# marcin-ochman/modular-slam

Measured on AMD Instinct MI355X. Metric: ORB keypoints extracted+matched /sec, 640×480 RGB-D, 1/2/4/8 GPU; HBM GB/s vs roofline, higher is better.
Workload: dtype u8

## Files before the change

modular-slam_amd/csrc/api.hip:

```cpp
#include "context.hpp"

#include <cfloat>
#include <climits>
#include <cmath>
#include <cstdio>
#include <cstring>
#include <cstdlib>
#include <algorithm>

using namespace mslam;

static thread_local std::string g_create_error;

#define ENTER(c)                                                                                                       \
    do                                                                                                                 \
    {                                                                                                                  \
        if(!(c))                                                                                                       \
            return MSLAM_HIP_E_INVALID;                                                                                \
        MSLAM_CHK(c, hipSetDevice((c)->p.device));                                                                     \
    } while(0)

static inline int cv_round_f(float v) { return (int)lrintf(v); }
static inline int cv_floor_f(float v)
{
// ... 1224 lines not shown
                exec = nullptr;
            if(rc)
                return rc;
            MSLAM_CHK(c, e);
            MSLAM_CHK(c, e_inst);
        }
        MSLAM_CHK(c, hipGraphLaunch(exec, c->stream));
    }
    else
    {
        rc = enqueue_detect(c, frame_src, 1);
        if(rc)
            return rc;
        rc = enqueue_results();
        if(rc)
            return rc;
    }
    MSLAM_CHK(c, hipEventRecord(c->out[c->cur].ev_detect, c->stream));
    c->n_last = 1;
    ++c->detect_seq;
    MSLAM_CHK(c, hipStreamSynchronize(c->stream));
    uint32_t flags;
    int32_t n;
    std::memcpy(&n, h, 4);
    std::memcpy(&flags, h + 4, 4);
    if(flags)
        return check_flags(c);
    *n_out = n;
    if(n > max_out)
        return fail(c, MSLAM_HIP_E_CAPACITY, "detect: max_out smaller than the number of keypoints");
    if(n == 0)
        return MSLAM_HIP_OK;
    std::memcpy(xy, h_xy, (size_t)n * 8);
    std::memcpy(desc, h_desc, (size_t)n * 32);
    if(octave)
        std::memcpy(octave, h_oct, (size_t)n * 4);
    if(angle)
        std::memcpy(angle, h_ang, (size_t)n * 4);
    if(response)
        std::memcpy(response, h_resp, (size_t)n * 4);
    return MSLAM_HIP_OK;
}

static int upload_ratio_table(mslam_hip_ctx* c, double ratio)
{
    if(ratio == c->ratio_cached)
        return MSLAM_HIP_OK;
    int32_t thr[257];
    for(int d1 = 0; d1 <= 256; ++d1)
    {
        int n = 0;
        for(int d0 = 0; d0 <= 256; ++d0)
            if((double)(float)d0 < ratio * (double)(float)d1)
                ++n;
            else
                break;
        thr[d1] = n;
    }
    MSLAM_CHK(c, hipStreamSynchronize(c->stream_m));
    MSLAM_CHK(c, hipMemcpyAsync(c->d_ratio_thr, thr, sizeof(thr), hipMemcpyHostToDevice, c->stream));
    MSLAM_CHK(c, hipStreamSynchronize(c->stream));
    c->ratio_cached = ratio;
    return MSLAM_HIP_OK;
}
__attribute__((visibility("hidden"))) int mslam_ratio_table(mslam_hip_ctx* c, double ratio) { return upload_ratio_table(c, ratio); }

int mslam_hip_match_batch_dev(mslam_hip_ctx* c, double ratio, int chain_previous)
{
    ENTER(c);
    if(c->n_last < 1)
        return fail(c, MSLAM_HIP_E_INVALID, "match_batch_dev: no detect batch to match");
    int rc = upload_ratio_table(c, ratio);
    if(rc)
        return rc;
    const size_t K = (size_t)c->p.max_keypoints;
    const int first = (chain_previous && c->have_prev) ? 0 : 1;
    const int n_pairs = c->n_last - first;
    c->match_seq = c->detect_seq;
    const bool own = c->overlap_match && !c->profiling;
    hipStream_t s = own ? c->stream_m : c->stream;
    if(own)
        MSLAM_CHK(c, hipStreamWaitEvent(s, c->out[c->cur].ev_detect, 0));
    if(first == 1)
        MSLAM_CHK(c, hipMemsetAsync(cur_out(c).mcount, 0, 4, s));
    if(n_pairs > 0)
    {
        MatchArgs m{};
        m.from_desc = cur_out(c).desc + (size_t)(first + 1) * K * 32;
        m.to_desc = cur_out(c).desc + (size_t)first * K * 32;
        m.from_stride = m.to_stride = (long long)K * 32;
        m.from_cnt = cur_out(c).count + first + 1;
        m.to_cnt = cur_out(c).count + first;
        m.cap = c->p.max_keypoints;
        m.cap_from = c->p.max_keypoints;
        m.popcount_only = c->matcher_kind == MSLAM_HIP_MATCHER_POPCOUNT;
        m.idx0 = cur_out(c).idx0 + (size_t)first * K;
        m.idx1 = cur_out(c).idx1 + (size_t)first * K;
        m.dist0 = cur_out(c).dist0 + (size_t)first * K;
        m.dist1 = cur_out(c).dist1 + (size_t)first * K;
        {
            StageScope t(c, "match_knn2", s);
            c->last_match_kernel = launch_match_knn2(m, n_pairs, s);
        }
        RatioArgs r{};
        r.idx0 = m.idx0;
        r.dist0 = m.dist0;
        r.dist1 = m.dist1;
        r.from_cnt = m.from_cnt;
        r.to_cnt = m.to_cnt;
        r.cap = m.cap;
        r.thr = c->d_ratio_thr;
        r.from_idx = cur_out(c).mfrom + (size_t)first * K;
        r.to_idx = cur_out(c).mto + (size_t)first * K;
        r.n_out = cur_out(c).mcount + first;
        {
            StageScope t(c, "ratio_compact", s);
            launch_ratio_compact(r, n_pairs, s);
        }
    }
    MSLAM_CHK(c, hipGetLastError());
    if(own)
    {
        MSLAM_CHK(c, hipEventRecord(c->out[c->cur].ev_match, s));
        c->out[c->cur].match_pending = true;
    }
    return MSLAM_HIP_OK;
}

constexpr int kHostMatchSlices = 8;
static int host_match_prepare(mslam_hip_ctx* c, const uint8_t* from_desc, int n_from, const uint8_t* to_desc, int n_to)
{
    if(n_from > c->hm_from_cap || n_to > c->hm_to_cap)
    {
        MSLAM_CHK(c, hipStreamSynchronize(c->stream));
        const int from_cap = std::max(n_from, std::max(c->hm_from_cap, 2048)), to_cap = std::max(n_to, std::max(c->hm_to_cap, 2048));
        c->hm_from_cap = c->hm_to_cap = 0;
        c->d_hm_to = nullptr;
        if(c->match_graph)
        {
            (void)hipGraphExecDestroy(c->match_graph);
            c->match_graph = nullptr;
        }
        MSLAM_CHK(c, c->d_hm_from.alloc((size_t)(from_cap + to_cap) * 32 + 16));
        MSLAM_CHK(c, c->d_hm_out.alloc((size_t)to_cap * 6 + 4));
        MSLAM_CHK(c, c->d_hm_partial.alloc((size_t)kHostMatchSlices * 2 * to_cap));
        MSLAM_CHK(c, c->h_hm.alloc((size_t)(from_cap + to_cap) * 32 + 16 + ((size_t)to_cap * 2 + 4) * 4));
        c->hm_from_cap = from_cap;
        c->hm_to_cap = to_cap;
    }
    c->d_hm_to = c->d_hm_from + (size_t)n_from * 32;
    if(n_from > 0)
        std::memcpy(c->h_hm, from_desc, (size_t)n_from * 32);
    std::memcpy(c->h_hm + (size_t)n_from * 32, to_desc, (size_t)n_to * 32);
    MSLAM_CHK(c, hipMemcpyAsync(c->d_hm_from, c->h_hm, (size_t)(n_from + n_to) * 32, hipMemcpyHostToDevice, c->stream));
    return MSLAM_HIP_OK;
}

static void host_match_args(mslam_hip_ctx* c, int n_from, int n_to, MatchArgs& m)
{
    const size_t cap = (size_t)c->hm_to_cap;
    m = MatchArgs{};
    m.from_desc = c->d_hm_from;
    m.to_desc = c->d_hm_to;
    m.n_from_fixed = n_from;
    m.n_to_fixed = n_to;
    m.cap = n_to;
    m.idx0 = c->d_hm_out;
// ... 388 lines not shown
```

modular-slam_amd/csrc/k_points.hip:

```cpp
#include "reloc.hpp"

#include <cfloat>

namespace mslam
{

struct Camera
{
    double cx, cy, inv_fx, inv_fy;
    float factor;
};

__global__ __launch_bounds__(256) void k_backproject(const uint16_t* __restrict__ depth, long long depth_stride, int w, int h,
                                                     Camera cam, const float* __restrict__ xy, long long xy_stride,
                                                     const int32_t* __restrict__ counts, int n_fixed, int cap,
                                                     double* __restrict__ xyz, uint8_t* __restrict__ valid)
{
    const int frame = blockIdx.y;
    const int n = min(counts ? counts[frame] : n_fixed, cap);
    const int i = blockIdx.x * 256 + threadIdx.x;
    if(i >= n)
        return;
    const float* p = xy + frame * xy_stride + 2 * (size_t)i;
    const double x = (double)p[0], y = (double)p[1];
    const bool inside = (x > -1.0) & (x < (double)w) & (y > -1.0) & (y < (double)h);
    float d = 0.f;
    if(inside)
        d = __fmul_rn((float)depth[frame * depth_stride + (size_t)w * (int)y + (int)x], cam.factor);
    const bool ok = d > FLT_EPSILON;
    const size_t o = (size_t)frame * cap + i;
    const double z = (double)d;
    xyz[3 * o] = ok ? (x - cam.cx) * z * cam.inv_fx : 0.0;
    xyz[3 * o + 1] = ok ? (y - cam.cy) * z * cam.inv_fy : 0.0;
    xyz[3 * o + 2] = ok ? z : 0.0;
    valid[o] = ok ? 1 : 0;
}

void launch_backproject(hipStream_t s, const uint16_t* d_depth, int width, int height, float factor, double fx, double fy, double cx,
                        double cy, const float* d_xy, int n, double* d_xyz, uint8_t* d_valid)
{
    const Camera cam{cx, cy, 1.0 / fx, 1.0 / fy, factor};
    hipLaunchKernelGGL(k_backproject, dim3((n + 255) / 256, 1), dim3(256), 0, s, d_depth, 0ll, width, height, cam, d_xy, 0ll, nullptr, n,
                       n, d_xyz, d_valid);
}

void launch_backproject_batch(hipStream_t s, const uint16_t* d_depth, int width, int height, float factor, double fx, double fy,
                              double cx, double cy, const float* d_xy, const int32_t* d_n, int stride, int n_frames, double* d_xyz,
                              uint8_t* d_valid)
{
    const Camera cam{cx, cy, 1.0 / fx, 1.0 / fy, factor};
    hipLaunchKernelGGL(k_backproject, dim3((stride + 255) / 256, n_frames), dim3(256), 0, s, d_depth, (long long)width * height, width,
                       height, cam, d_xy, (long long)stride * 2, d_n, 0, stride, d_xyz, d_valid);
}

}

using namespace mslam;

__global__ __launch_bounds__(1024) void k_pack_plan(const int32_t* __restrict__ count, const int32_t* __restrict__ mcount, int n_frames,
                                                    int cap, int with_points, unsigned long long capacity_bytes, uint8_t* __restrict__ out,
                                                    uint32_t* __restrict__ flags)
{
    __shared__ uint32_t wsum[2][16];
    __shared__ uint32_t carry[2];
    const int tid = threadIdx.x, lane = tid & 63, wave = tid >> 6;
    mslam_hip_packed_header* h = reinterpret_cast<mslam_hip_packed_header*>(out);
    const unsigned long long hdr = (sizeof(mslam_hip_packed_header) + 15) & ~15ull;
    const unsigned long long tab = (((unsigned long long)(n_frames + 1) * 4) + 15) & ~15ull;
    const bool room_for_tables = capacity_bytes >= hdr + 2 * tab;
    int32_t* kp_off = reinterpret_cast<int32_t*>(out + hdr);
    int32_t* m_off = reinterpret_cast<int32_t*>(out + hdr + tab);
    if(tid < 2)
        carry[tid] = 0;
    __syncthreads();
    for(int base = 0; base < n_frames; base += 1024)
    {
        const int t = base + tid;
        uint32_t v[2] = {t < n_frames ? (uint32_t)min(max(count[t], 0), cap) : 0u, (t < n_frames && mcount) ? (uint32_t)min(max(mcount[t], 0), cap) : 0u};
        uint32_t inc[2];
#pragma unroll
        for(int k = 0; k < 2; ++k)
        {
            uint32_t x = v[k];
            for(int o = 1; o < 64; o <<= 1)
            {
                const uint32_t y = (uint32_t)__shfl_up((int)x, o);
                x += lane >= o ? y : 0u;
            }
            inc[k] = x;
            if(lane == 63)
                wsum[k][wave] = x;
        }
        __syncthreads();
#pragma unroll
        for(int k = 0; k < 2; ++k)
        {
            uint32_t pre = carry[k];
            for(int w = 0; w < wave; ++w)
                pre += wsum[k][w];
            if(t < n_frames && room_for_tables)
                (k == 0 ? kp_off : m_off)[t] = (int32_t)(pre + inc[k] - v[k]);
        }
        __syncthreads();
        if(tid < 2)
        {
            uint32_t tot = carry[tid];
            for(int w = 0; w < 16; ++w)
                tot += wsum[tid][w];
            carry[tid] = tot;
        }
        __syncthreads();
    }
    if(tid == 0)
    {
        const unsigned long long nk = carry[0], nm = carry[1];
        auto al = [](unsigned long long x) { return (x + 15) & ~15ull; };
        unsigned long long o = hdr + 2 * tab;
        mslam_hip_packed_header hh;
        hh.n_frames = n_frames, hh.total_keypoints = (int32_t)nk, hh.total_matches = (int32_t)nm, hh.with_points = with_points;
        hh.off_kp_offset = hdr, hh.off_match_offset = hdr + tab;
        hh.off_xy = o, o = al(o + nk * 8);
        hh.off_desc = o, o = al(o + nk * 32);
        hh.off_octave = o, o = al(o + nk * 4);
        hh.off_angle = o, o = al(o + nk * 4);
        hh.off_response = o, o = al(o + nk * 4);
        hh.off_xyz = o, o = al(o + (with_points ? nk * 24 : 0));
        hh.off_valid = o, o = al(o + (with_points ? nk : 0));
        hh.off_match_from = o, o = al(o + nm * 4);
        hh.off_match_to = o, o = al(o + nm * 4);
        hh.bytes = o;
        hh.fits = o <= capacity_bytes ? 1 : 0;
        hh.pad = 0;
        if(capacity_bytes >= sizeof(hh))
            *h = hh;
// ... 4 lines not shown
    }
}

__global__ __launch_bounds__(256) void k_pack_copy(const float* __restrict__ xy, const uint8_t* __restrict__ desc, const int32_t* __restrict__ octave,
                                                   const float* __restrict__ angle, const float* __restrict__ response,
                                                   const double* __restrict__ xyz, const uint8_t* __restrict__ valid,
                                                   const int32_t* __restrict__ mfrom, const int32_t* __restrict__ mto, int cap,
                                                   uint8_t* __restrict__ out)
{
    const mslam_hip_packed_header* h = reinterpret_cast<const mslam_hip_packed_header*>(out);
    if(!h->fits)
        return;
    const int t = blockIdx.x, tid = blockIdx.y * 256 + threadIdx.x, nt = gridDim.y * 256;
    const int32_t* kp_off = reinterpret_cast<const int32_t*>(out + h->off_kp_offset);
    const int32_t* m_off = reinterpret_cast<const int32_t*>(out + h->off_match_offset);
    const size_t k0 = (size_t)kp_off[t], m0 = (size_t)m_off[t];
    const int n = kp_off[t + 1] - kp_off[t], m = m_off[t + 1] - m_off[t];
    const size_t f = (size_t)t * cap;
    uint2* o_xy = reinterpret_cast<uint2*>(out + h->off_xy) + k0;
    uint2* o_desc = reinterpret_cast<uint2*>(out + h->off_desc) + 4 * k0;
    uint32_t* o_oct = reinterpret_cast<uint32_t*>(out + h->off_octave) + k0;
    uint32_t* o_ang = reinterpret_cast<uint32_t*>(out + h->off_angle) + k0;
    uint32_t* o_resp = reinterpret_cast<uint32_t*>(out + h->off_response) + k0;
    for(int i = tid; i < 4 * n; i += nt)
        o_desc[i] = reinterpret_cast<const uint2*>(desc)[4 * f + i];
    for(int i = tid; i < n; i += nt)
    {
        o_xy[i] = reinterpret_cast<const uint2*>(xy)[f + i];
        o_oct[i] = reinterpret_cast<const uint32_t*>(octave)[f + i];
        o_ang[i] = reinterpret_cast<const uint32_t*>(angle)[f + i];
        o_resp[i] = reinterpret_cast<const uint32_t*>(response)[f + i];
    }
    if(h->with_points)
    {
        double* o_xyz = reinterpret_cast<double*>(out + h->off_xyz) + 3 * k0;
        uint8_t* o_val = out + h->off_valid + k0;
        for(int i = tid; i < 3 * n; i += nt)
            o_xyz[i] = xyz[3 * f + i];
        for(int i = tid; i < n; i += nt)
            o_val[i] = valid[f + i];
    }
    uint32_t* o_mf = reinterpret_cast<uint32_t*>(out + h->off_match_from) + m0;
    uint32_t* o_mt = reinterpret_cast<uint32_t*>(out + h->off_match_to) + m0;
    for(int i = tid; i < m; i += nt)
    {
        o_mf[i] = reinterpret_cast<const uint32_t*>(mfrom)[f + i];
        o_mt[i] = reinterpret_cast<const uint32_t*>(mto)[f + i];
    }
}

static bool bad_focal(double f)
{
    return f == 0.0 || f != f;
}

static int ensure_points(mslam_hip_ctx* c)
{
    if(c->d_xyz)
        return MSLAM_HIP_OK;
    const size_t n = (size_t)c->p.max_batch * c->p.max_keypoints;
    MSLAM_CHK(c, c->d_xyz.alloc(n * 3));
    MSLAM_CHK(c, c->d_valid.alloc(n));
    return MSLAM_HIP_OK;
}

extern "C" {

int mslam_hip_backproject_batch_dev(mslam_hip_ctx* c, const uint16_t* d_depth, float factor, double fx, double fy,
                                    double cx, double cy)
{
    if(!c)
        return MSLAM_HIP_E_INVALID;
    if(!d_depth || bad_focal(fx) || bad_focal(fy))
        return fail(c, MSLAM_HIP_E_INVALID, "backproject_batch_dev: bad argument");
    if(c->n_last < 1)
        return fail(c, MSLAM_HIP_E_INVALID, "backproject_batch_dev: no detect batch");
    MSLAM_CHK(c, hipSetDevice(c->p.device));
    int rc = ensure_points(c);
    if(rc)
        return rc;
    const size_t K = (size_t)c->p.max_keypoints;
    const Camera cam{cx, cy, 1.0 / fx, 1.0 / fy, factor};
    StageScope t(c, "backproject");
    dim3 grid((c->p.max_keypoints + 255) / 256, c->n_last);
    hipLaunchKernelGGL(k_backproject, grid, dim3(256), 0, c->stream, d_depth, (long long)c->p.width * c->p.height,
                       c->p.width, c->p.height, cam, cur_out(c).xy + K * 2, (long long)K * 2, cur_out(c).count + 1, 0,
                       c->p.max_keypoints, c->d_xyz, c->d_valid);
    MSLAM_CHK(c, hipGetLastError());
    c->points_seq = c->detect_seq;
    return MSLAM_HIP_OK;
}

int mslam_hip_pack_batch_dev(mslam_hip_ctx* c, void* out, size_t capacity_bytes, int with_points)
{
    if(!c)
        return MSLAM_HIP_E_INVALID;
    if(!out || capacity_bytes < sizeof(mslam_hip_packed_header))
        return fail(c, MSLAM_HIP_E_INVALID, "pack_batch_dev: no output buffer (at least the header must fit)");
    if(c->n_last < 1)
        return fail(c, MSLAM_HIP_E_INVALID, "pack_batch_dev: no detect batch");
    if(with_points && (!c->d_xyz || c->points_seq != c->detect_seq))
        return fail(c, MSLAM_HIP_E_INVALID, "pack_batch_dev: with_points, but the last detect batch has not been back-projected");
    MSLAM_CHK(c, hipSetDevice(c->p.device));
    int rc = mslam_hip_join_matcher(c);
    if(rc)
        return rc;
    const size_t K = (size_t)c->p.max_keypoints;
    const mslam_out_set& o = cur_out(c);
    const int32_t* mcount = c->match_seq == c->detect_seq ? o.mcount : nullptr;
    hipLaunchKernelGGL(k_pack_plan, dim3(1), dim3(1024), 0, c->stream, o.count + 1, mcount, c->n_last, c->p.max_keypoints,
                       with_points ? 1 : 0, (unsigned long long)capacity_bytes, static_cast<uint8_t*>(out), c->d_flags);
    hipLaunchKernelGGL(k_pack_copy, dim3(c->n_last, 4), dim3(256), 0, c->stream, o.xy + K * 2, o.desc + K * 32, o.octave + K,
                       o.angle + K, o.response + K, c->d_xyz, c->d_valid, o.mfrom, o.mto, c->p.max_keypoints,
                       static_cast<uint8_t*>(out));
    MSLAM_CHK(c, hipGetLastError());
    return MSLAM_HIP_OK;
}

size_t mslam_hip_packed_capacity(const mslam_hip_ctx* c, int n_frames, int with_points)
{
    if(!c || n_frames < 0)
        return 0;
    const size_t K = (size_t)c->p.max_keypoints, n = (size_t)n_frames;
    return 256 + 2 * (((n + 1) * 4 + 15) & ~(size_t)15) + n * K * (8 + 32 + 4 + 4 + 4 + (with_points ? 25 : 0) + 8) + 16 * 16;
}

int mslam_hip_get_points_view(mslam_hip_ctx* c, mslam_hip_points_view* v)
{
    if(!c || !v)
        return MSLAM_HIP_E_INVALID;
    int rc = ensure_points(c);
    if(rc)
        return rc;
    v->capacity = c->p.max_keypoints;
    v->xyz = c->d_xyz;
    v->valid = c->d_valid;
    return MSLAM_HIP_OK;
}

int mslam_hip_backproject(mslam_hip_ctx* c, const uint16_t* depth, int width, int height, float factor, double fx,
                          double fy, double cx, double cy, const float* xy, int n, double* xyz, uint8_t* valid)
{
    if(!c)
        return MSLAM_HIP_E_INVALID;
    if(!depth || width <= 0 || height <= 0 || n < 0 || (n > 0 && (!xy || !xyz || !valid)) || bad_focal(fx) || bad_focal(fy))
        return fail(c, MSLAM_HIP_E_INVALID, "backproject: bad argument");
    if(n == 0)
        return MSLAM_HIP_OK;
    MSLAM_CHK(c, hipSetDevice(c->p.device));
    DevBuf<uint16_t> d_depth;
    DevBuf<float> d_xy;
    DevBuf<double> d_xyz;
    DevBuf<uint8_t> d_valid;
    const size_t npx = (size_t)width * height;
    hipStream_t s = c->stream;
    hipError_t e = d_depth.alloc(npx);
    if(e == hipSuccess) e = d_xy.alloc((size_t)n * 2);
    if(e == hipSuccess) e = d_xyz.alloc((size_t)n * 3);
    if(e == hipSuccess) e = d_valid.alloc((size_t)n);
    if(e == hipSuccess) e = hipMemcpyAsync(d_depth, depth, npx * 2, hipMemcpyHostToDevice, s);
    if(e == hipSuccess) e = hipMemcpyAsync(d_xy, xy, (size_t)n * 8, hipMemcpyHostToDevice, s);
    if(e == hipSuccess)
    {
        const Camera cam{cx, cy, 1.0 / fx, 1.0 / fy, factor};
        hipLaunchKernelGGL(k_backproject, dim3((n + 255) / 256, 1), dim3(256), 0, s, d_depth, 0ll, width, height, cam, d_xy,
                           0ll, nullptr, n, n, d_xyz, d_valid);
        e = hipGetLastError();
    }
    if(e == hipSuccess) e = hipMemcpyAsync(xyz, d_xyz, (size_t)n * 24, hipMemcpyDeviceToHost, s);
    if(e == hipSuccess) e = hipMemcpyAsync(valid, d_valid, (size_t)n, hipMemcpyDeviceToHost, s);
    if(e == hipSuccess) e = hipStreamSynchronize(s);
    if(e != hipSuccess)
    {
        c->err = std::string("backproject: ") + hipGetErrorString(e);
        return MSLAM_HIP_E_RUNTIME;
    }
    return MSLAM_HIP_OK;
}

}
```

modular-slam_amd/csrc/k_quadtree.hip:

```cpp
#include "common.hpp"
#include <algorithm>
#include <cstdlib>

namespace mslam
{

constexpr int QT = 512;
constexpr int kSmallKp = 512, kSmallQT = 256;
constexpr int kMidKp = 1024, kMidQT = 512;
constexpr int kLdsKp = 2048;
constexpr int kMaxCellsPerLevel = 2048;
constexpr int kBigNodes = 4096;
constexpr int kBigKp = 12288;
constexpr int kBigMinPixels = 400000;
constexpr int kMaxInitNodes = 64;
constexpr int kDirectKp = 1024, kDirectQT = 256, kDirectSlots = 1365, kDirectMaxDepth = 10;
constexpr int kMaxPasses = 40;

struct Scan
{
    uint32_t wsum[QT / 64];
};

__device__ __forceinline__ uint32_t wave_incl_scan(uint32_t v)
{
    int x = (int)v;
    x += __builtin_amdgcn_update_dpp(0, x, 0x111, 0xF, 0xF, true);
    x += __builtin_amdgcn_update_dpp(0, x, 0x112, 0xF, 0xF, true);
    x += __builtin_amdgcn_update_dpp(0, x, 0x114, 0xF, 0xE, true);
    x += __builtin_amdgcn_update_dpp(0, x, 0x118, 0xF, 0xC, true);
    x += __builtin_amdgcn_update_dpp(0, x, 0x142, 0xA, 0xF, true);
    x += __builtin_amdgcn_update_dpp(0, x, 0x143, 0xC, 0xF, true);
    return (uint32_t)x;
}

template <int NT>
__device__ __forceinline__ uint32_t block_excl_scan(uint32_t v, Scan& s, uint32_t& total)
{
    const int lane = threadIdx.x & 63, wave = threadIdx.x >> 6;
    const uint32_t inc = wave_incl_scan(v);
    if(lane == 63)
        s.wsum[wave] = inc;
    __syncthreads();
    uint32_t base = 0, tot = 0;
#pragma unroll
    for(int w = 0; w < NT / 64; ++w)
    {
        const uint32_t x = s.wsum[w];
        if(w < wave)
            base += x;
        tot += x;
    }
    __syncthreads();
    total = tot;
    return base + inc - v;
}

template <int NT>
__device__ __forceinline__ void block_excl_scan2(uint32_t a, uint32_t b, Scan& s, Scan& s2, uint32_t& exa, uint32_t& exb,
                                                 uint32_t& tota, uint32_t& totb)
{
    const int lane = threadIdx.x & 63, wave = threadIdx.x >> 6;
    const uint32_t ia = wave_incl_scan(a), ib = wave_incl_scan(b);
    if(lane == 63)
    {
        s.wsum[wave] = ia;
        s2.wsum[wave] = ib;
    }
    __syncthreads();
    uint32_t ba = 0, bb = 0, ta = 0, tb = 0;
#pragma unroll
    for(int w = 0; w < NT / 64; ++w)
    {
        const uint32_t x = s.wsum[w], y = s2.wsum[w];
        if(w < wave)
        {
            ba += x;
            bb += y;
        }
        ta += x;
        tb += y;
    }
    __syncthreads();
    tota = ta;
    totb = tb;
    exa = ba + ia - a;
    exb = bb + ib - b;
}

__device__ __forceinline__ uint32_t ld_atomic(const uint32_t* p)
{
    return __hip_atomic_load(p, __ATOMIC_RELAXED, __HIP_MEMORY_SCOPE_AGENT);
}

__device__ __forceinline__ void unpack_node(uint2 b, int& bx, int& by, int& ex, int& ey)
{
    bx = (int)(b.x & 0xFFFF), by = (int)(b.x >> 16), ex = (int)(b.y & 0xFFFF), ey = (int)(b.y >> 16);
}
__device__ __forceinline__ uint2 pack_node(int bx, int by, int ex, int ey)
// ... 195 lines not shown
                continue;
            const uint32_t info = ninfo[pos];
            uint32_t np;
            if(info & 1u)
            {
                int bx, by, ex, ey;
                unpack_node(nodes[pos], bx, by, ex, ey);
                const int cx = bx + ((ex - bx + 1) >> 1), cy = by + ((ey - by + 1) >> 1);
                const uint32_t p = cand[k];
                const int c = (cx <= kp_x(p) ? 1 : 0) + (cy <= kp_y(p) ? 2 : 0);
                np = T - 1 - (uint32_t)nbase[pos] - (uint32_t)__popc((info >> 1) & ((1u << c) - 1u));
            }
            else
                np = T + (uint32_t)nbase[pos];
            kp_node[k] = (idx_t)np;
        }
        __syncthreads();
        {
            uint2* t = nodes; nodes = nodes2; nodes2 = t;
            idx_t* u = ncnt; ncnt = ncnt2; ncnt2 = u;
        }
        const uint32_t n2 = T + U;
        const bool same = n2 == n;
        n = n2;
        if(same)
        {
            converged = true;
            break;
        }
    }
    if(!converged && n > 0 && tid == 0)
        atomicOr(a.flags, kFlagQuadNoConverge);

    for(uint32_t pos = tid; pos < n; pos += NT)
        best[pos] = 0;
    __syncthreads();
    for(uint32_t k = tid; k < N; k += NT)
    {
        const uint32_t pos = kp_node[k];
        if(pos == kNoNode)
            continue;
        atomicMax(&best[pos], ((uint32_t)kp_score(cand[k]) << 24) | (0xFFFFFFu - k));
    }
    __syncthreads();
    for(uint32_t pos = tid; pos < n; pos += NT)
    {
        const uint32_t k = 0xFFFFFFu - ((S::kLds ? best[pos] : ld_atomic(&best[pos])) & 0xFFFFFFu);
        sel[pos] = cand[k];
    }
    if(tid == 0)
        a.sel_cnt[slot] = n;
    return true;
}

template <int NT>
__device__ __forceinline__ uint32_t quad_cell_offsets(const uint32_t* ccnt, int n_cells, uint32_t* cell_off, Scan& scan)
{
    const int tid = threadIdx.x;
    uint32_t running = 0;
    for(int base = 0; base < n_cells; base += NT)
    {
        const int i = base + tid;
        const uint32_t v = i < n_cells ? ccnt[i] : 0u;
        uint32_t tot;
        const uint32_t ex = block_excl_scan<NT>(v, scan, tot);
        if(i < n_cells)
            cell_off[i] = running + ex;
        running += tot;
    }
    if(tid == 0)
        cell_off[n_cells] = running;
    __syncthreads();
    return running;
}

__device__ __forceinline__ int quad_class(uint32_t N, int n_cells, unsigned classes)
{
    if((classes & 1u) && N <= (uint32_t)kSmallKp && n_cells <= 2 * kSmallKp - 1)
        return 0;
    if((classes & 2u) && N <= (uint32_t)kMidKp && n_cells <= 2 * kMidKp - 1)
        return 1;
    return 2;
}
template <int KP, int NT, int CLS>
__global__ __launch_bounds__(NT) __attribute__((amdgpu_waves_per_eu(CLS == 2 ? 4 : 8))) void k_quadtree(Geometry g, QuadArgs a, unsigned big_levels, unsigned direct_levels)
{
    __shared__ Scan scan, scan2;
    __shared__ uint32_t l_cand[KP];
    __shared__ uint2 l_nodes_a[KP], l_nodes_b[KP];
    __shared__ uint32_t l_cc[KP * 2];
    __shared__ uint16_t l_kp_node[KP], l_ncnt_a[KP], l_ncnt_b[KP], l_nbase[KP];
    __shared__ uint8_t l_ninfo[KP];
    __shared__ uint32_t init_cnt[kMaxInitNodes];
    __shared__ uint32_t init_pos[kMaxInitNodes];
    __shared__ uint32_t sh_n;
    constexpr int kCellsFit = 2 * KP - 1;
    static_assert(CLS != 2 || kCellsFit >= kMaxCellsPerLevel, "cell offsets must fit");
    const unsigned classes = big_levels >> 30;
    uint32_t* cell_off = reinterpret_cast<uint32_t*>(l_nodes_b);

    const int level = (int)((blockIdx.x + blockIdx.y) % (unsigned)g.n_levels);
    const size_t frame = blockIdx.y + g.frame0;
    const LevelGeom& lv = g.lv[level];
    const int tid = threadIdx.x;
    const size_t slot = frame * g.n_levels + level;
    const size_t cap = (size_t)a.cand_cap;
    uint32_t* cand = a.cand + slot * cap;
    uint32_t* sel = a.sel + slot * cap;

    const int n_cells = lv.n_cells;
    if(n_cells > kCellsFit)
        return;
    const uint32_t* ccnt = a.cell_cnt + frame * g.n_cells + lv.cell_base;
    const uint32_t N = quad_cell_offsets<NT>(ccnt, n_cells, cell_off, scan);
    if(((direct_levels >> level) & 1u) && N <= (uint32_t)kDirectKp)
        return;
    if(quad_class(N, n_cells, classes) != CLS)
        return;
    if(N > (uint32_t)a.cand_cap)
    {
        if(tid == 0)
        {
            atomicOr(a.flags, kFlagCandOverflow);
            a.cand_cnt[slot] = 0;
            a.sel_cnt[slot] = 0;
        }
        return;
    }
    if(tid == 0)
        a.cand_cnt[slot] = N;
    if(N == 0)
    {
        if(tid == 0)
            a.sel_cnt[slot] = 0;
        return;
    }
    if(N <= (uint32_t)KP)
        quad_run<LdsStore, NT>(g, a, lv, frame, slot, tid, N, n_cells, cell_off, l_cand, cand, l_kp_node, l_nodes_a, l_nodes_b,
                               l_ncnt_a, l_ncnt_b, l_ninfo, l_nbase, l_cc, l_cc, sel, scan, scan2, init_cnt, init_pos, sh_n);
    else if((big_levels >> level) & 1u)
        return;
    else
        quad_run<GlobalStore, NT>(g, a, lv, frame, slot, tid, N, n_cells, cell_off, cand, cand, a.kp_node + slot * cap,
                                  a.nodes_a + slot * cap, a.nodes_b + slot * cap, a.ncnt_a + slot * cap,
                                  a.ncnt_b + slot * cap, a.ninfo + slot * cap, a.best + slot * cap,
                                  a.child_cnt + slot * cap * 4, a.best + slot * cap, sel, scan, scan2, init_cnt, init_pos,
                                  sh_n);
}

__global__ __launch_bounds__(QT) void k_quadtree_big(Geometry g, QuadArgs a, unsigned big_levels)
{
    extern __shared__ __attribute__((aligned(16))) uint8_t big_lds[];
    __shared__ Scan scan, scan2;
    __shared__ uint32_t init_cnt[kMaxInitNodes];
    __shared__ uint32_t init_pos[kMaxInitNodes];
    __shared__ uint32_t sh_n;
    uint2* l_nodes_a = reinterpret_cast<uint2*>(big_lds);
    uint2* l_nodes_b = l_nodes_a + kBigNodes;
    uint32_t* l_cc = reinterpret_cast<uint32_t*>(l_nodes_b + kBigNodes);
    uint16_t* l_kp_node = reinterpret_cast<uint16_t*>(l_cc + 2 * kBigNodes);
    uint16_t* l_ncnt_a = l_kp_node + kBigKp;
    uint16_t* l_ncnt_b = l_ncnt_a + kBigNodes;
    uint16_t* l_nbase = l_ncnt_b + kBigNodes;
    uint8_t* l_ninfo = reinterpret_cast<uint8_t*>(l_nbase + kBigNodes);
    static_assert(kBigNodes * sizeof(uint2) >= (kMaxCellsPerLevel + 1) * sizeof(uint32_t), "cell offsets must fit");
    uint32_t* cell_off = reinterpret_cast<uint32_t*>(l_nodes_b);

    int level = 0;
    {
        unsigned m = big_levels;
        const unsigned which = (blockIdx.x + blockIdx.y) % gridDim.x;
        for(unsigned i = 0; i < which; ++i)
            m &= m - 1;
        level = __ffs((int)m) - 1;
    }
    const size_t frame = blockIdx.y + g.frame0;
    const LevelGeom& lv = g.lv[level];
    const int tid = threadIdx.x;
    const size_t slot = frame * g.n_levels + level;
    const size_t cap = (size_t)a.cand_cap;
    uint32_t* cand = a.cand + slot * cap;
    uint32_t* sel = a.sel + slot * cap;
    const int n_cells = lv.n_cells;
    const uint32_t* ccnt = a.cell_cnt + frame * g.n_cells + lv.cell_base;
    const uint32_t N = quad_cell_offsets<QT>(ccnt, n_cells, cell_off, scan);
    if(N <= (uint32_t)kLdsKp || N > (uint32_t)a.cand_cap)
        return;
    bool done = false;
    if(N <= (uint32_t)kBigKp)
        done = quad_run<BigStore, QT>(g, a, lv, frame, slot, tid, N, n_cells, cell_off, cand, cand, l_kp_node, l_nodes_a, l_nodes_b,
                                  l_ncnt_a, l_ncnt_b, l_ninfo, l_nbase, l_cc, l_cc, sel, scan, scan2, init_cnt, init_pos, sh_n);
    if(!done)
    {
        __syncthreads();
        quad_cell_offsets<QT>(ccnt, n_cells, cell_off, scan);
        quad_run<GlobalStore, QT>(g, a, lv, frame, slot, tid, N, n_cells, cell_off, cand, cand, a.kp_node + slot * cap,
                              a.nodes_a + slot * cap, a.nodes_b + slot * cap, a.ncnt_a + slot * cap,
                              a.ncnt_b + slot * cap, a.ninfo + slot * cap, a.best + slot * cap,
                              a.child_cnt + slot * cap * 4, a.best + slot * cap, sel, scan, scan2, init_cnt, init_pos,
                              sh_n);
    }
}

template <int SLOTS>
struct DirectTable
{
    uint32_t cnt[(SLOTS + 1) / 2];
    uint32_t best[SLOTS];
    uint8_t flag[SLOTS];
};

__device__ __forceinline__ uint32_t direct_block_start(uint32_t n_init, int d) { return n_init * (((1u << (2 * d)) - 1u) / 3u); }

template <int KP, int SLOTS, int NT>
__global__ __launch_bounds__(NT) __attribute__((amdgpu_waves_per_eu(8))) void k_quadtree_direct(Geometry g, QuadArgs a, unsigned direct_levels)
{
    constexpr int PER = KP / NT;
    static_assert(KP % NT == 0 && KP == kDirectKp, "instance shape");
    __shared__ Scan scan;
    __shared__ uint32_t l_cand[KP];
    __shared__ DirectTable<SLOTS> t;
    __shared__ uint32_t tot[2 * (kDirectMaxDepth + 2)];

    const int level = (int)((blockIdx.x + blockIdx.y) % (unsigned)g.n_levels);
    if(!((direct_levels >> level) & 1u))
        return;
    const size_t frame = blockIdx.y + g.frame0;
    const LevelGeom& lv = g.lv[level];
    const int tid = threadIdx.x;
    const size_t slot = frame * g.n_levels + level;
    const size_t cap = (size_t)a.cand_cap;
    uint32_t* g_cand = a.cand + slot * cap;
    uint32_t* sel = a.sel + slot * cap;
    const int D = lv.qdepth;
    const uint32_t n_init = (uint32_t)(lv.nxg * lv.nyg);
    const uint32_t n_slots = direct_block_start(n_init, D + 1);

    for(uint32_t i = tid; i < (n_slots + 1) / 2; i += NT)
        t.cnt[i] = 0;
    for(uint32_t i = tid; i < n_slots; i += NT)
        t.flag[i] = 0;
    if(tid < 2 * (kDirectMaxDepth + 2))
        tot[tid] = 0;

    const int n_cells = lv.n_cells;
    uint32_t* cell_off = t.best;
    const uint32_t* ccnt = a.cell_cnt + frame * g.n_cells + lv.cell_base;
    const uint32_t N = quad_cell_offsets<NT>(ccnt, n_cells, cell_off, scan);
    if(N > (uint32_t)KP)
        return;
    if(N > (uint32_t)a.cand_cap)
    {
        if(tid == 0)
        {
            atomicOr(a.flags, kFlagCandOverflow);
            a.cand_cnt[slot] = 0;
            a.sel_cnt[slot] = 0;
        }
        return;
    }
    if(tid == 0)
        a.cand_cnt[slot] = N;
    if(N == 0)
    {
        if(tid == 0)
            a.sel_cnt[slot] = 0;
        return;
    }

    const uint32_t* ckp = a.cell_kp + (frame * g.n_cells + lv.cell_base) * (size_t)kCellCap;
    const float sf = lv.scale;
    const float min_size_f = (float)a.min_size;
    uint32_t path[PER];
#pragma unroll
    for(int i = 0; i < PER; ++i)
    {
        const uint32_t k = (uint32_t)(tid + i * NT);
        path[i] = ~0u;
        if(k >= N)
            continue;
        int lo = 0, hi = n_cells - 1;
        while(lo < hi)
        {
            const int mid = (lo + hi + 1) >> 1;
            if(cell_off[mid] <= k)
                lo = mid;
            else
                hi = mid - 1;
        }
        const uint32_t p = ckp[(size_t)lo * kCellCap + (k - cell_off[lo])];
        l_cand[k] = p;
        g_cand[k] = p;
        const int x = kp_x(p), y = kp_y(p);
        const unsigned ix = (unsigned)((double)(float)x / lv.delta_x);
        const unsigned iy = (unsigned)((double)(float)y / lv.delta_y);
        const unsigned idx = ix + iy * (unsigned)lv.nxg;
        if(idx >= n_init)
            continue;
        int bx = (int)(lv.delta_x * ix), by = (int)(lv.delta_y * iy);
        int ex = (int)(lv.delta_x * (ix + 1)), ey = (int)(lv.delta_y * (iy + 1));
        uint32_t q = idx;
        int d = 0;
        for(;;)
        {
            const uint32_t s = direct_block_start(n_init, d) + q;
            atomicAdd(&t.cnt[s >> 1], 1u << (16 * (s & 1u)));
            const unsigned area = (unsigned)((ex - bx) * (ey - by));
            if(__fmul_rn(__fmul_rn((float)area, sf), sf) <= min_size_f || d == D)
            {
                t.flag[s] = 1;
                break;
            }
            const int cx = bx + ((ex - bx + 1) >> 1), cy = by + ((ey - by + 1) >> 1);
            const bool right = cx <= x, low = cy <= y;
            bx = right ? cx : bx, ex = right ? ex : cx;
            by = low ? cy : by, ey = low ? ey : cy;
            q = (q << 2) | (right ? 1u : 0u) | (low ? 2u : 0u);
            ++d;
        }
        path[i] = ((uint32_t)d << 24) | q;
    }
    __syncthreads();

    for(int d = 0; d <= D; ++d)
    {
        const uint32_t start = direct_block_start(n_init, d), n_d = n_init << (2 * d);
        const uint32_t pstart = direct_block_start(n_init, d > 0 ? d - 1 : 0);
        uint32_t kd = 0, md = 0;
        for(uint32_t base = 0; base < n_d; base += NT)
        {
            const uint32_t q = base + tid;
            bool keep = false, open = false;
            if(q < n_d)
            {
                const uint32_t s = start + q, ps = pstart + (q >> 2);
                const uint32_t c = (t.cnt[s >> 1] >> (16 * (s & 1u))) & 0xFFFFu;
                const uint32_t pc = d > 0 ? (t.cnt[ps >> 1] >> (16 * (ps & 1u))) & 0xFFFFu : 2u;
                const bool real = c > 0 && pc >= 2;
                keep = real && (c == 1 || t.flag[s] != 0);
                open = real && !keep;
                t.flag[s] = keep ? 1 : open ? 2 : 0;
                t.best[s] = 0;
            }
            kd += (uint32_t)__popcll(__ballot(keep));
            md += (uint32_t)__popcll(__ballot(open));
        }
        if((tid & 63) == 0 && (kd | md) != 0)
        {
            atomicAdd(&tot[2 * d], kd);
            atomicAdd(&tot[2 * d + 1], md);
        }
    }
    __syncthreads();
    int P = 1;
    while(tot[2 * P] + tot[2 * P + 1] != tot[2 * P - 1])
        ++P;
    const int top = P < D ? P : D;

#pragma unroll
    for(int i = 0; i < PER; ++i)
    {
        if(path[i] == ~0u)
            continue;
        const uint32_t k = (uint32_t)(tid + i * NT);
        const int dk = (int)(path[i] >> 24);
        const uint32_t q = path[i] & 0xFFFFFFu;
        const int last = dk < top ? dk : top;
        uint32_t leaf = 0;
        for(int d = 0; d <= last; ++d)
        {
            leaf = direct_block_start(n_init, d) + (q >> (2 * (dk - d)));
            if(t.flag[leaf] == 1)
                break;
        }
        atomicMax(&t.best[leaf], ((uint32_t)kp_score(l_cand[k]) << 24) | (0xFFFFFFu - k));
    }
    __syncthreads();

    const uint32_t n_entries = direct_block_start(n_init, top + 1);
    const uint32_t per = (n_entries + NT - 1) / NT;
    const uint32_t e0 = (uint32_t)tid * per, e1 = e0 + per < n_entries ? e0 + per : n_entries;
    auto entry_slot = [&](uint32_t e, bool& is_leaf) {
        int d = top;
        uint32_t n_d = n_init << (2 * d);
        while(e >= n_d)
        {
            e -= n_d;
            --d;
            n_d >>= 2;
        }
        const uint32_t bits = 2u * (uint32_t)d, low_mask = (1u << bits) - 1u;
        uint32_t i0 = e >> bits;
        if(d & 1)
            i0 = n_init - 1u - i0;
        const uint32_t s = direct_block_start(n_init, d) + ((i0 << bits) | ((e ^ 0x33333333u) & low_mask));
        const uint32_t f = t.flag[s];
        is_leaf = f == 1 || (f == 2 && d == P);
        return s;
    };
    uint32_t mine = 0;
    for(uint32_t e = e0; e < e1; ++e)
    {
        bool is_leaf;
        entry_slot(e, is_leaf);
        mine += is_leaf ? 1u : 0u;
    }
    uint32_t n_leaves;
    uint32_t r = block_excl_scan<NT>(mine, scan, n_leaves);
    for(uint32_t e = e0; e < e1 && mine != 0; ++e)
    {
        bool is_leaf;
        const uint32_t s = entry_slot(e, is_leaf);
        if(is_leaf)
            sel[r++] = l_cand[0xFFFFFFu - (t.best[s] & 0xFFFFFFu)];
    }
    if(tid == 0)
        a.sel_cnt[slot] = n_leaves;
}

unsigned quad_direct_levels(const Geometry& g)
{
    const char* env = getenv("MSLAM_HIP_QUAD_DIRECT");
    const bool on = !env || atoi(env) != 0;
    unsigned m = 0;
    for(int l = 0; on && l < g.n_levels; ++l)
    {
        const LevelGeom& lv = g.lv[l];
        if(lv.qdepth < 0 || lv.qdepth > kDirectMaxDepth || lv.n_cells + 1 > kDirectSlots)
            continue;
        const long long slots = (long long)lv.nxg * lv.nyg * (((1ll << (2 * (lv.qdepth + 1))) - 1) / 3);
        if(slots <= kDirectSlots)
            m |= 1u << l;
    }
    return m;
}

int quad_depth_bound(const LevelGeom& lv, unsigned min_size)
{
    int dx = 0, dy = 0;
    for(int iy = 0; iy < lv.nyg; ++iy)
        for(int ix = 0; ix < lv.nxg; ++ix)
        {
            dx = std::max(dx, (int)(lv.delta_x * (ix + 1)) - (int)(lv.delta_x * ix));
            dy = std::max(dy, (int)(lv.delta_y * (iy + 1)) - (int)(lv.delta_y * iy));
        }
    for(int d = 0; d <= 15; ++d)
    {
        const unsigned area = (unsigned)(dx * dy);
        const float scaled = (float)area * lv.scale;
        if(scaled * lv.scale <= (float)min_size)
            return d;
        if(dx <= 1 && dy <= 1)
            break;
        dx = (dx + 1) >> 1, dy = (dy + 1) >> 1;
    }
    return -1;
}

void launch_quadtree(const Geometry& g, const QuadArgs& a, int frame0, int n_frames, hipStream_t s)
{
    dim3 grid(g.n_levels, n_frames);
    Geometry gg = g;
    gg.frame0 = frame0;
    unsigned big_levels = 0;
    for(int l = 0; l < g.n_levels; ++l)
        if(g.lv[l].w * g.lv[l].h > kBigMinPixels)
            big_levels |= 1u << l;
    static const unsigned classes_env = [] { const char* e = getenv("MSLAM_HIP_QUAD_CLASSES"); return e ? (unsigned)atoi(e) & 3u : 3u; }();
    const unsigned direct = quad_direct_levels(g);
    const bool all_direct = direct == (g.n_levels >= 32 ? ~0u : (1u << g.n_levels) - 1u);
    const unsigned classes = n_frames < 8 || all_direct ? 0u : classes_env;
    const unsigned bl = big_levels | (classes << 30);
    if(direct != 0)
        hipLaunchKernelGGL((k_quadtree_direct<kDirectKp, kDirectSlots, kDirectQT>), grid, dim3(kDirectQT), 0, s, gg, a, direct);
    hipLaunchKernelGGL((k_quadtree<kLdsKp, QT, 2>), grid, dim3(QT), 0, s, gg, a, bl, direct);
    if(classes & 2u)
        hipLaunchKernelGGL((k_quadtree<kMidKp, kMidQT, 1>), grid, dim3(kMidQT), 0, s, gg, a, bl, direct);
    if(classes & 1u)
        hipLaunchKernelGGL((k_quadtree<kSmallKp, kSmallQT, 0>), grid, dim3(kSmallQT), 0, s, gg, a, bl, direct);
    if(big_levels != 0)
    {
        constexpr size_t lds = (size_t)kBigNodes * (8 + 8 + 8 + 2 + 2 + 2 + 1) + (size_t)kBigKp * 2;
        static const bool attr = [] {
            return hipFuncSetAttribute((const void*)k_quadtree_big, hipFuncAttributeMaxDynamicSharedMemorySize, (int)lds) == hipSuccess;
        }();
        (void)attr;
        hipLaunchKernelGGL(k_quadtree_big, dim3((unsigned)__builtin_popcount(big_levels), n_frames), dim3(QT), lds, s, gg, a,
                           big_levels);
    }
}

}
```

Measured before the change: 665.7 million.

## Restructure backproject kernel with grid-stride unrolling and LDS-staged vector stores

Rewrites the back-projection kernel as a grid-stride loop with a capped grid and four-way unrolled loads of keypoints and depths. Each wave stages its xyz triples in shared memory so they can be written out as coalesced 16-byte stores instead of three strided 8-byte stores. Separately, the match-count memset is replaced with a small zeroing kernel launch. The changes add per-wave barriers and alignment branches, and backprojection is likely a minor stage of the overall pipeline.

```diff
diff --git a/modular-slam_amd/csrc/api.hip b/modular-slam_amd/csrc/api.hip
--- a/modular-slam_amd/csrc/api.hip
+++ b/modular-slam_amd/csrc/api.hip
@@ -1330,7 +1330,7 @@
     if(own)
         MSLAM_CHK(c, hipStreamWaitEvent(s, c->out[c->cur].ev_detect, 0));
     if(first == 1)
-        MSLAM_CHK(c, hipMemsetAsync(cur_out(c).mcount, 0, 4, s));
+        launch_zero_u32(reinterpret_cast<uint32_t*>(static_cast<int32_t*>(cur_out(c).mcount)), 1, s);
     if(n_pairs > 0)
     {
         MatchArgs m{};
diff --git a/modular-slam_amd/csrc/k_points.hip b/modular-slam_amd/csrc/k_points.hip
--- a/modular-slam_amd/csrc/k_points.hip
+++ b/modular-slam_amd/csrc/k_points.hip
@@ -1,5 +1,6 @@
 #include "reloc.hpp"
 
+#include <algorithm>
 #include <cfloat>
 
 namespace mslam
@@ -10,37 +11,95 @@
     double cx, cy, inv_fx, inv_fy;
     float factor;
 };
+
+constexpr int kBpUnroll = 4;
+constexpr int kBpFillWorkgroups = 2048;
+
+static dim3 backproject_grid(int cap, int n_frames)
+{
+    const int full = (cap + 255) / 256;
+    return dim3((unsigned)std::max(1, std::min(full, kBpFillWorkgroups / std::max(n_frames, 1))), (unsigned)n_frames);
+}
 
 __global__ __launch_bounds__(256) void k_backproject(const uint16_t* __restrict__ depth, long long depth_stride, int w, int h,
                                                      Camera cam, const float* __restrict__ xy, long long xy_stride,
                                                      const int32_t* __restrict__ counts, int n_fixed, int cap,
                                                      double* __restrict__ xyz, uint8_t* __restrict__ valid)
 {
+    __shared__ __attribute__((aligned(16))) double stage[4][64 * 3];
     const int frame = blockIdx.y;
     const int n = min(counts ? counts[frame] : n_fixed, cap);
-    const int i = blockIdx.x * 256 + threadIdx.x;
-    if(i >= n)
-        return;
-    const float* p = xy + frame * xy_stride + 2 * (size_t)i;
-    const double x = (double)p[0], y = (double)p[1];
-    const bool inside = (x > -1.0) & (x < (double)w) & (y > -1.0) & (y < (double)h);
-    float d = 0.f;
-    if(inside)
-        d = __fmul_rn((float)depth[frame * depth_stride + (size_t)w * (int)y + (int)x], cam.factor);
-    const bool ok = d > FLT_EPSILON;
-    const size_t o = (size_t)frame * cap + i;
-    const double z = (double)d;
-    xyz[3 * o] = ok ? (x - cam.cx) * z * cam.inv_fx : 0.0;
-    xyz[3 * o + 1] = ok ? (y - cam.cy) * z * cam.inv_fy : 0.0;
-    xyz[3 * o + 2] = ok ? z : 0.0;
-    valid[o] = ok ? 1 : 0;
+    const int lane = threadIdx.x & 63, wave = __builtin_amdgcn_readfirstlane(threadIdx.x >> 6);
+    const int stride = gridDim.x * 256;
+    const float* fxy = xy + frame * xy_stride;
+    const uint16_t* fdepth = depth + frame * depth_stride;
+    const size_t fo = (size_t)frame * cap;
+    for(int i0 = blockIdx.x * 256 + wave * 64; i0 < n; i0 += kBpUnroll * stride)
+    {
+        double x[kBpUnroll], y[kBpUnroll];
+        bool inside[kBpUnroll];
+        uint16_t raw[kBpUnroll];
+#pragma unroll
+        for(int u = 0; u < kBpUnroll; ++u)
+        {
+            const float* p = fxy + 2 * (size_t)min(i0 + u * stride + lane, n - 1);
+            x[u] = (double)p[0], y[u] = (double)p[1];
+        }
+#pragma unroll
+        for(int u = 0; u < kBpUnroll; ++u)
+        {
+            inside[u] = (x[u] > -1.0) & (x[u] < (double)w) & (y[u] > -1.0) & (y[u] < (double)h);
+            const int px = inside[u] ? (int)x[u] : 0, py = inside[u] ? (int)y[u] : 0;
+            raw[u] = fdepth[(size_t)w * py + px];
+        }
+#pragma unroll
+        for(int u = 0; u < kBpUnroll; ++u)
+        {
+            const int b = i0 + u * stride;
+            if(b >= n)
+                break;
+            const int i = b + lane;
+            const float d = inside[u] ? __fmul_rn((float)raw[u], cam.factor) : 0.f;
+            const bool ok = d > FLT_EPSILON;
+            const double z = (double)d;
+            const double X = ok ? (x[u] - cam.cx) * z * cam.inv_fx : 0.0;
+            const double Y = ok ? (y[u] - cam.cy) * z * cam.inv_fy : 0.0;
+            const double Z = ok ? z : 0.0;
+            if(i < n)
+                valid[fo + i] = ok ? 1 : 0;
+            double* out = xyz + 3 * (fo + b);
+            if(reinterpret_cast<uintptr_t>(out) & 15)
+            {
+                if(i < n)
+                    out[3 * lane] = X, out[3 * lane + 1] = Y, out[3 * lane + 2] = Z;
+                continue;
+            }
+            double* st = stage[wave];
+            st[3 * lane] = X, st[3 * lane + 1] = Y, st[3 * lane + 2] = Z;
+            __builtin_amdgcn_fence(__ATOMIC_RELEASE, "wavefront");
+            __builtin_amdgcn_wave_barrier();
+            __builtin_amdgcn_fence(__ATOMIC_ACQUIRE, "wavefront");
+            const double2 lo = reinterpret_cast<const double2*>(st)[lane];
+            const double hi = st[128 + lane];
+            const int bytes = 24 * min(64, n - b);
+            char* o = reinterpret_cast<char*>(out);
+            if(16 * lane + 16 <= bytes)
+                *reinterpret_cast<double2*>(o + 16 * lane) = lo;
+            else if(16 * lane + 8 <= bytes)
+                *reinterpret_cast<double*>(o + 16 * lane) = lo.x;
+            if(1024 + 8 * lane + 8 <= bytes)
+                *reinterpret_cast<double*>(o + 1024 + 8 * lane) = hi;
+            __builtin_amdgcn_fence(__ATOMIC_RELEASE, "wavefront");
+            __builtin_amdgcn_wave_barrier();
+        }
+    }
 }
 
 void launch_backproject(hipStream_t s, const uint16_t* d_depth, int width, int height, float factor, double fx, double fy, double cx,
                         double cy, const float* d_xy, int n, double* d_xyz, uint8_t* d_valid)
 {
     const Camera cam{cx, cy, 1.0 / fx, 1.0 / fy, factor};
-    hipLaunchKernelGGL(k_backproject, dim3((n + 255) / 256, 1), dim3(256), 0, s, d_depth, 0ll, width, height, cam, d_xy, 0ll, nullptr, n,
+    hipLaunchKernelGGL(k_backproject, backproject_grid(n, 1), dim3(256), 0, s, d_depth, 0ll, width, height, cam, d_xy, 0ll, nullptr, n,
                        n, d_xyz, d_valid);
 }
 
@@ -49,7 +108,7 @@
                               uint8_t* d_valid)
 {
     const Camera cam{cx, cy, 1.0 / fx, 1.0 / fy, factor};
-    hipLaunchKernelGGL(k_backproject, dim3((stride + 255) / 256, n_frames), dim3(256), 0, s, d_depth, (long long)width * height, width,
+    hipLaunchKernelGGL(k_backproject, backproject_grid(stride, n_frames), dim3(256), 0, s, d_depth, (long long)width * height, width,
                        height, cam, d_xy, (long long)stride * 2, d_n, 0, stride, d_xyz, d_valid);
 }
 
@@ -220,7 +279,7 @@
     const size_t K = (size_t)c->p.max_keypoints;
     const Camera cam{cx, cy, 1.0 / fx, 1.0 / fy, factor};
     StageScope t(c, "backproject");
-    dim3 grid((c->p.max_keypoints + 255) / 256, c->n_last);
+    const dim3 grid = backproject_grid(c->p.max_keypoints, c->n_last);
     hipLaunchKernelGGL(k_backproject, grid, dim3(256), 0, c->stream, d_depth, (long long)c->p.width * c->p.height,
                        c->p.width, c->p.height, cam, cur_out(c).xy + K * 2, (long long)K * 2, cur_out(c).count + 1, 0,
                        c->p.max_keypoints, c->d_xyz, c->d_valid);
@@ -301,7 +360,7 @@
     if(e == hipSuccess)
     {
         const Camera cam{cx, cy, 1.0 / fx, 1.0 / fy, factor};
-        hipLaunchKernelGGL(k_backproject, dim3((n + 255) / 256, 1), dim3(256), 0, s, d_depth, 0ll, width, height, cam, d_xy,
+        hipLaunchKernelGGL(k_backproject, backproject_grid(n, 1), dim3(256), 0, s, d_depth, 0ll, width, height, cam, d_xy,
                            0ll, nullptr, n, n, d_xyz, d_valid);
         e = hipGetLastError();
     }
```

After: 666.2 million, median of 6. No clear change (+0.1%).

## Extend direct quadtree kernel to handle overflow keypoints and skip list-based launches

Applied to the files above, without the earlier changes.

The direct-table quadtree kernel now accepts levels with more than 1024 candidates, up to 65535, on non-big levels. Keypoints past the LDS capacity are gathered to global memory, counted in the table, and then re-walked and voted in a strided loop. When every level is handled by the direct path, the host skips launching the list-based quadtree kernels entirely. This removes redundant kernel launches and the fallback to the heavier multi-pass kernel, at the cost of recomputing tree walks and reading global memory for overflow points.

```diff
diff --git a/modular-slam_amd/csrc/k_quadtree.hip b/modular-slam_amd/csrc/k_quadtree.hip
--- a/modular-slam_amd/csrc/k_quadtree.hip
+++ b/modular-slam_amd/csrc/k_quadtree.hip
@@ -1,6 +1,7 @@
 #include "common.hpp"
 #include <algorithm>
 #include <cstdlib>
+#include <type_traits>
 
 namespace mslam
 {
@@ -15,6 +16,7 @@
 constexpr int kBigMinPixels = 400000;
 constexpr int kMaxInitNodes = 64;
 constexpr int kDirectKp = 1024, kDirectQT = 256, kDirectSlots = 1365, kDirectMaxDepth = 10;
+constexpr uint32_t kDirectMaxN = 65535;
 constexpr int kMaxPasses = 40;
 
 struct Scan
@@ -376,8 +378,12 @@
         return 1;
     return 2;
 }
+__device__ __forceinline__ bool quad_direct_takes(bool sweeps, uint32_t N, uint32_t cand_cap)
+{
+    return sweeps ? N <= kDirectMaxN || N > cand_cap : N <= (uint32_t)kDirectKp;
+}
 template <int KP, int NT, int CLS>
-__global__ __launch_bounds__(NT) __attribute__((amdgpu_waves_per_eu(CLS == 2 ? 4 : 8))) void k_quadtree(Geometry g, QuadArgs a, unsigned big_levels, unsigned direct_levels)
+__global__ __launch_bounds__(NT) __attribute__((amdgpu_waves_per_eu(CLS == 2 ? 4 : 8))) void k_quadtree(Geometry g, QuadArgs a, unsigned big_levels, unsigned direct_levels, unsigned sweep_levels)
 {
     __shared__ Scan scan, scan2;
     __shared__ uint32_t l_cand[KP];
@@ -407,7 +413,7 @@
         return;
     const uint32_t* ccnt = a.cell_cnt + frame * g.n_cells + lv.cell_base;
     const uint32_t N = quad_cell_offsets<NT>(ccnt, n_cells, cell_off, scan);
-    if(((direct_levels >> level) & 1u) && N <= (uint32_t)kDirectKp)
+    if(((direct_levels >> level) & 1u) && quad_direct_takes((sweep_levels >> level) & 1u, N, (uint32_t)a.cand_cap))
         return;
     if(quad_class(N, n_cells, classes) != CLS)
         return;
@@ -506,8 +512,74 @@
 
 __device__ __forceinline__ uint32_t direct_block_start(uint32_t n_init, int d) { return n_init * (((1u << (2 * d)) - 1u) / 3u); }
 
+__device__ __forceinline__ uint32_t direct_gather(const uint32_t* ckp, const uint32_t* cell_off, int n_cells, uint32_t k)
+{
+    int lo = 0, hi = n_cells - 1;
+    while(lo < hi)
+    {
+        const int mid = (lo + hi + 1) >> 1;
+        if(cell_off[mid] <= k)
+            lo = mid;
+        else
+            hi = mid - 1;
+    }
+    return ckp[(size_t)lo * kCellCap + (k - cell_off[lo])];
+}
+
+template <bool COUNT, int SLOTS>
+__device__ __forceinline__ uint32_t direct_walk(uint32_t p, const LevelGeom& lv, uint32_t n_init, int D, float sf,
+                                                float min_size_f, DirectTable<SLOTS>& t)
+{
+    const int x = kp_x(p), y = kp_y(p);
+    const unsigned ix = (unsigned)((double)(float)x / lv.delta_x);
+    const unsigned iy = (unsigned)((double)(float)y / lv.delta_y);
+    const unsigned idx = ix + iy * (unsigned)lv.nxg;
+    if(idx >= n_init)
+        return ~0u;
+    int bx = (int)(lv.delta_x * ix), by = (int)(lv.delta_y * iy);
+    int ex = (int)(lv.delta_x * (ix + 1)), ey = (int)(lv.delta_y * (iy + 1));
+    uint32_t q = idx;
+    int d = 0;
+    for(;;)
+    {
+        const uint32_t s = direct_block_start(n_init, d) + q;
+        if(COUNT)
+            atomicAdd(&t.cnt[s >> 1], 1u << (16 * (s & 1u)));
+        const unsigned area = (unsigned)((ex - bx) * (ey - by));
+        if(__fmul_rn(__fmul_rn((float)area, sf), sf) <= min_size_f || d == D)
+        {
+            if(COUNT)
+                t.flag[s] = 1;
+            break;
+        }
+        const int cx = bx + ((ex - bx + 1) >> 1), cy = by + ((ey - by + 1) >> 1);
+        const bool right = cx <= x, low = cy <= y;
+        bx = right ? cx : bx, ex = right ? ex : cx;
+        by = low ? cy : by, ey = low ? ey : cy;
+        q = (q << 2) | (right ? 1u : 0u) | (low ? 2u : 0u);
+        ++d;
+    }
+    return ((uint32_t)d << 24) | q;
+}
+
+template <int SLOTS>
+__device__ __forceinline__ void direct_vote(uint32_t path, uint32_t k, uint32_t p, uint32_t n_init, int top, DirectTable<SLOTS>& t)
+{
+    const int dk = (int)(path >> 24);
+    const uint32_t q = path & 0xFFFFFFu;
+    const int last = dk < top ? dk : top;
+    uint32_t leaf = 0;
+    for(int d = 0; d <= last; ++d)
+    {
+        leaf = direct_block_start(n_init, d) + (q >> (2 * (dk - d)));
+        if(t.flag[leaf] == 1)
+            break;
+    }
+    atomicMax(&t.best[leaf], ((uint32_t)kp_score(p) << 24) | (0xFFFFFFu - k));
+}
+
 template <int KP, int SLOTS, int NT>
-__global__ __launch_bounds__(NT) __attribute__((amdgpu_waves_per_eu(8))) void k_quadtree_direct(Geometry g, QuadArgs a, unsigned direct_levels)
+__global__ __launch_bounds__(NT) __attribute__((amdgpu_waves_per_eu(8))) void k_quadtree_direct(Geometry g, QuadArgs a, unsigned direct_levels, unsigned sweep_levels)
 {
     constexpr int PER = KP / NT;
     static_assert(KP % NT == 0 && KP == kDirectKp, "instance shape");
@@ -541,7 +613,7 @@
     uint32_t* cell_off = t.best;
     const uint32_t* ccnt = a.cell_cnt + frame * g.n_cells + lv.cell_base;
     const uint32_t N = quad_cell_offsets<NT>(ccnt, n_cells, cell_off, scan);
-    if(N > (uint32_t)KP)
+    if(!quad_direct_takes((sweep_levels >> level) & 1u, N, (uint32_t)a.cand_cap))
         return;
     if(N > (uint32_t)a.cand_cap)
     {
@@ -573,47 +645,19 @@
         path[i] = ~0u;
         if(k >= N)
             continue;
-        int lo = 0, hi = n_cells - 1;
-        while(lo < hi)
-        {
-            const int mid = (lo + hi + 1) >> 1;
-            if(cell_off[mid] <= k)
-                lo = mid;
-            else
-                hi = mid - 1;
-        }
-        const uint32_t p = ckp[(size_t)lo * kCellCap + (k - cell_off[lo])];
+        const uint32_t p = direct_gather(ckp, cell_off, n_cells, k);
         l_cand[k] = p;
         g_cand[k] = p;
-        const int x = kp_x(p), y = kp_y(p);
-        const unsigned ix = (unsigned)((double)(float)x / lv.delta_x);
-        const unsigned iy = (unsigned)((double)(float)y / lv.delta_y);
-        const unsigned idx = ix + iy * (unsigned)lv.nxg;
-        if(idx >= n_init)
-            continue;
-        int bx = (int)(lv.delta_x * ix), by = (int)(lv.delta_y * iy);
-        int ex = (int)(lv.delta_x * (ix + 1)), ey = (int)(lv.delta_y * (iy + 1));
-        uint32_t q = idx;
-        int d = 0;
-        for(;;)
-        {
-            const uint32_t s = direct_block_start(n_init, d) + q;
-            atomicAdd(&t.cnt[s >> 1], 1u << (16 * (s & 1u)));
-            const unsigned area = (unsigned)((ex - bx) * (ey - by));
-            if(__fmul_rn(__fmul_rn((float)area, sf), sf) <= min_size_f || d == D)
-            {
-                t.flag[s] = 1;
-                break;
-            }
-            const int cx = bx + ((ex - bx + 1) >> 1), cy = by + ((ey - by + 1) >> 1);
-            const bool right = cx <= x, low = cy <= y;
-            bx = right ? cx : bx, ex = right ? ex : cx;
-            by = low ? cy : by, ey = low ? ey : cy;
-            q = (q << 2) | (right ? 1u : 0u) | (low ? 2u : 0u);
-            ++d;
-        }
-        path[i] = ((uint32_t)d << 24) | q;
-    }
+        path[i] = direct_walk<true>(p, lv, n_init, D, sf, min_size_f, t);
+    }
+    const bool more = N > (uint32_t)KP;
+    if(more)
+        for(uint32_t k = (uint32_t)(KP + tid); k < N; k += NT)
+        {
+            const uint32_t p = direct_gather(ckp, cell_off, n_cells, k);
+            g_cand[k] = p;
+            direct_walk<true>(p, lv, n_init, D, sf, min_size_f, t);
+        }
     __syncthreads();
 
     for(int d = 0; d <= D; ++d)
@@ -657,18 +701,16 @@
         if(path[i] == ~0u)
             continue;
         const uint32_t k = (uint32_t)(tid + i * NT);
-        const int dk = (int)(path[i] >> 24);
-        const uint32_t q = path[i] & 0xFFFFFFu;
-        const int last = dk < top ? dk : top;
-        uint32_t leaf = 0;
-        for(int d = 0; d <= last; ++d)
-        {
-            leaf = direct_block_start(n_init, d) + (q >> (2 * (dk - d)));
-            if(t.flag[leaf] == 1)
-                break;
-        }
-        atomicMax(&t.best[leaf], ((uint32_t)kp_score(l_cand[k]) << 24) | (0xFFFFFFu - k));
-    }
+        direct_vote(path[i], k, l_cand[k], n_init, top, t);
+    }
+    if(more)
+        for(uint32_t k = (uint32_t)(KP + tid); k < N; k += NT)
+        {
+            const uint32_t p = ld_atomic(&g_cand[k]);
+            const uint32_t pk = direct_walk<false>(p, lv, n_init, D, sf, min_size_f, t);
+            if(pk != ~0u)
+                direct_vote(pk, k, p, n_init, top, t);
+        }
     __syncthreads();
 
     const uint32_t n_entries = direct_block_start(n_init, top + 1);
@@ -701,13 +743,21 @@
     }
     uint32_t n_leaves;
     uint32_t r = block_excl_scan<NT>(mine, scan, n_leaves);
-    for(uint32_t e = e0; e < e1 && mine != 0; ++e)
-    {
-        bool is_leaf;
-        const uint32_t s = entry_slot(e, is_leaf);
-        if(is_leaf)
-            sel[r++] = l_cand[0xFFFFFFu - (t.best[s] & 0xFFFFFFu)];
-    }
+    auto emit = [&](auto later) {
+        for(uint32_t e = e0; e < e1 && mine != 0; ++e)
+        {
+            bool is_leaf;
+            const uint32_t s = entry_slot(e, is_leaf);
+            if(!is_leaf)
+                continue;
+            const uint32_t k = 0xFFFFFFu - (t.best[s] & 0xFFFFFFu);
+            sel[r++] = decltype(later)::value && k >= (uint32_t)KP ? ld_atomic(&g_cand[k]) : l_cand[k];
+        }
+    };
+    if(more)
+        emit(std::true_type{});
+    else
+        emit(std::false_type{});
     if(tid == 0)
         a.sel_cnt[slot] = n_leaves;
 }
@@ -762,16 +812,20 @@
             big_levels |= 1u << l;
     static const unsigned classes_env = [] { const char* e = getenv("MSLAM_HIP_QUAD_CLASSES"); return e ? (unsigned)atoi(e) & 3u : 3u; }();
     const unsigned direct = quad_direct_levels(g);
+    const unsigned sweep = direct & ~big_levels;
     const bool all_direct = direct == (g.n_levels >= 32 ? ~0u : (1u << g.n_levels) - 1u);
+    const bool list_passes = !all_direct || sweep != direct || (uint32_t)a.cand_cap > kDirectMaxN;
     const unsigned classes = n_frames < 8 || all_direct ? 0u : classes_env;
     const unsigned bl = big_levels | (classes << 30);
     if(direct != 0)
-        hipLaunchKernelGGL((k_quadtree_direct<kDirectKp, kDirectSlots, kDirectQT>), grid, dim3(kDirectQT), 0, s, gg, a, direct);
-    hipLaunchKernelGGL((k_quadtree<kLdsKp, QT, 2>), grid, dim3(QT), 0, s, gg, a, bl, direct);
+        hipLaunchKernelGGL((k_quadtree_direct<kDirectKp, kDirectSlots, kDirectQT>), grid, dim3(kDirectQT), 0, s, gg, a, direct, sweep);
+    if(!list_passes)
+        return;
+    hipLaunchKernelGGL((k_quadtree<kLdsKp, QT, 2>), grid, dim3(QT), 0, s, gg, a, bl, direct, sweep);
     if(classes & 2u)
-        hipLaunchKernelGGL((k_quadtree<kMidKp, kMidQT, 1>), grid, dim3(kMidQT), 0, s, gg, a, bl, direct);
+        hipLaunchKernelGGL((k_quadtree<kMidKp, kMidQT, 1>), grid, dim3(kMidQT), 0, s, gg, a, bl, direct, sweep);
     if(classes & 1u)
-        hipLaunchKernelGGL((k_quadtree<kSmallKp, kSmallQT, 0>), grid, dim3(kSmallQT), 0, s, gg, a, bl, direct);
+        hipLaunchKernelGGL((k_quadtree<kSmallKp, kSmallQT, 0>), grid, dim3(kSmallQT), 0, s, gg, a, bl, direct, sweep);
     if(big_levels != 0)
     {
         constexpr size_t lds = (size_t)kBigNodes * (8 + 8 + 8 + 2 + 2 + 2 + 1) + (size_t)kBigKp * 2;
```

Measured after the change: 666.5 million before, 669.6 million after (median of 6 runs). No clear change (+0.5%).
